# alazarteka/Self-Forcing

Measured on AMD Instinct MI355X. Metric: decoded frames/sec/node, Wan-1.3B 832x480 4-step AR rollout, higher is better.
Workload: dtype bf16

## Files before the change

### self-forcing_amd/csrc/gemm_bf16.hip

```cpp
#include <type_traits>
#include "sf_common.h"
#include "lds_dma.h"
#include "../../include/sf_hip.h"

namespace {

constexpr int BM = 128, BN = 128, BK = 64;
constexpr int GEMM_THREADS = 256;
constexpr int TILE_BYTES = BM * BK * 2;
constexpr int STAGE_BYTES = 2 * TILE_BYTES;
constexpr int GEMM_LDS = 2 * STAGE_BYTES;

struct GemmP {
  const bf16_t* a;
  const bf16_t* w;
  const bf16_t* bias;
  bf16_t* out;
  const bf16_t* resid;
  const bf16_t* gate_mod;
  const bf16_t* gate_e0;
  long gate_group_stride;
  int rows_per_group;
  int M, N, K, lda, ldw, ldo, ldr;
  int tiles_m, tiles_n;
  long a_bs, w_bs, o_bs, r_bs;
  const float* a_scale;
  const float* w_scale;
  int rows_per_seg;
};

typedef int i32x4 __attribute__((ext_vector_type(4)));
typedef int i32x8 __attribute__((ext_vector_type(8)));

__device__ __forceinline__ f32x4 mfma_f8(const bf16x8& w0, const bf16x8& w1, const bf16x8& x0, const bf16x8& x1, const f32x4& acc) {
  const i32x8 wv = __builtin_shufflevector(__builtin_bit_cast(i32x4, w0), __builtin_bit_cast(i32x4, w1), 0, 1, 2, 3, 4, 5, 6, 7);
  const i32x8 xv = __builtin_shufflevector(__builtin_bit_cast(i32x4, x0), __builtin_bit_cast(i32x4, x1), 0, 1, 2, 3, 4, 5, 6, 7);
  return __builtin_amdgcn_mfma_scale_f32_16x16x128_f8f6f4(wv, xv, acc, 0, 0, 0, 127, 0, 127);
}

template <int MT>
__device__ __forceinline__ void fp8_scale_acc(const GemmP& p, f32x4 (&acc)[MT][4], int m_base, int n_base, int lane) {
  f32x4 ws[4];
#pragma unroll
  for (int nt = 0; nt < 4; ++nt) ws[nt] = *reinterpret_cast<const f32x4*>(p.w_scale + min(n_base + nt * 16 + (lane >> 4) * 4, p.N - 4));
#pragma unroll
  for (int mt = 0; mt < MT; ++mt) {
    const float sa = p.a_scale[min(m_base + mt * 16 + (lane & 15), p.M - 1) / p.rows_per_seg];
#pragma unroll
    for (int nt = 0; nt < 4; ++nt)
#pragma unroll
      for (int j = 0; j < 4; ++j) acc[mt][nt][j] = acc[mt][nt][j] * (sa * ws[nt][j]);
  }
}

template <int EPI>
__device__ __forceinline__ bf16x4 epi_apply(const GemmP& p, const f32x4& a4, int m, int n, const bf16_t* e0row) {
  float y[4];
#pragma unroll
  for (int j = 0; j < 4; ++j) y[j] = a4[j];
  if (p.bias) {
    const bf16x4 b = *reinterpret_cast<const bf16x4*>(p.bias + n);
#pragma unroll
    for (int j = 0; j < 4; ++j) y[j] += (float)b[j];
  }
  if (EPI == SF_EPI_BIAS_GELU) {
#pragma unroll
    for (int j = 0; j < 4; ++j) y[j] = gelu_tanh_f(y[j]);
  }
  if (EPI == SF_EPI_BIAS_GATE_RESID) {
    const bf16x4 gm = *reinterpret_cast<const bf16x4*>(p.gate_mod + n);
    const bf16x4 ge = *reinterpret_cast<const bf16x4*>(e0row + n);
#pragma unroll
    for (int j = 0; j < 4; ++j) y[j] *= (float)(bf16_t)((float)gm[j] + (float)ge[j]);
  }
  if (EPI == SF_EPI_BIAS_RESID || EPI == SF_EPI_BIAS_GATE_RESID) {
    const bf16x4 rv = *reinterpret_cast<const bf16x4*>(p.resid + (long)m * p.ldr + n);
#pragma unroll
    for (int j = 0; j < 4; ++j) y[j] += (float)rv[j];
  }
  bf16x4 o;
#pragma unroll
  for (int j = 0; j < 4; ++j) o[j] = (bf16_t)y[j];
  return o;
}

template <int EPI, int MT>
__device__ __forceinline__ void gemm_epilogue(const GemmP& p, f32x4 (&acc)[MT][4], int mrow, int ncol) {
#pragma unroll
  for (int mt = 0; mt < MT; ++mt) {
    const int m = mrow + mt * 16;
    if (m >= p.M) continue;
    const bf16_t* e0row = nullptr;
    if (EPI == SF_EPI_BIAS_GATE_RESID) e0row = p.gate_e0 + (long)(m / p.rows_per_group) * p.gate_group_stride;
#pragma unroll
    for (int nt = 0; nt < 4; ++nt) {
      const int n = ncol + nt * 16;
      if (n >= p.N) continue;
      if (EPI == SF_EPI_F32) {
        *reinterpret_cast<f32x4*>(reinterpret_cast<float*>(p.out) + (long)m * p.ldo + n) = acc[mt][nt];
        continue;
      }
      *reinterpret_cast<bf16x4*>(p.out + (long)m * p.ldo + n) = epi_apply<EPI>(p, acc[mt][nt], m, n, e0row);
    }
  }
}

template <int EPI>
__device__ __forceinline__ bf16x4 epi_math(const f32x4& a4, const bf16x4& b, const bf16x4& gm, const bf16x4& ge, const bf16x4& rv) {
  float y[4];
#pragma unroll
  for (int j = 0; j < 4; ++j) y[j] = a4[j] + (float)b[j];
  if (EPI == SF_EPI_BIAS_GELU) {
#pragma unroll
    for (int j = 0; j < 4; ++j) y[j] = gelu_tanh_f(y[j]);
  }
  if (EPI == SF_EPI_BIAS_GATE_RESID) {
#pragma unroll
    for (int j = 0; j < 4; ++j) y[j] *= (float)(bf16_t)((float)gm[j] + (float)ge[j]);
  }
  if (EPI == SF_EPI_BIAS_RESID || EPI == SF_EPI_BIAS_GATE_RESID) {
#pragma unroll
    for (int j = 0; j < 4; ++j) y[j] += (float)rv[j];
  }
  bf16x4 o;
#pragma unroll
  for (int j = 0; j < 4; ++j) o[j] = (bf16_t)y[j];
  return o;
}

template <int EPI, int MT>
__device__ __forceinline__ void gemm_epilogue_lds(const GemmP& p, f32x4 (&acc)[MT][4], int m_base, int n_base, char* wbuf, int lane) {
  const int r16 = lane & 15, cg = lane >> 4;
  constexpr bool GATE = EPI == SF_EPI_BIAS_GATE_RESID;
  constexpr bool RESID = EPI == SF_EPI_BIAS_RESID || EPI == SF_EPI_BIAS_GATE_RESID;
  const bf16x4 zero4 = {(bf16_t)0.f, (bf16_t)0.f, (bf16_t)0.f, (bf16_t)0.f};
  int ncol[4];
  bf16x4 bias_v[4], gm_v[4];
#pragma unroll
  for (int nt = 0; nt < 4; ++nt) {
    ncol[nt] = min(n_base + nt * 16 + cg * 4, p.N - 4);
    bias_v[nt] = zero4;
    gm_v[nt] = zero4;
  }
  if (p.bias) {
#pragma unroll
    for (int nt = 0; nt < 4; ++nt) bias_v[nt] = *reinterpret_cast<const bf16x4*>(p.bias + ncol[nt]);
  }
  if (GATE) {
#pragma unroll
    for (int nt = 0; nt < 4; ++nt) gm_v[nt] = *reinterpret_cast<const bf16x4*>(p.gate_mod + ncol[nt]);
  }
  constexpr int MB = 4;
#pragma unroll
  for (int m0 = 0; m0 < MT; m0 += MB) {
    bf16x4 rv[MB][4], ge[MB][4];
#pragma unroll
    for (int i = 0; i < MB; ++i) {
      if (m0 + i >= MT) break;
      const int m = min(m_base + (m0 + i) * 16 + r16, p.M - 1);
      const bf16_t* e0row = GATE ? p.gate_e0 + (long)(m / p.rows_per_group) * p.gate_group_stride : nullptr;
#pragma unroll
      for (int nt = 0; nt < 4; ++nt) {
        rv[i][nt] = RESID ? *reinterpret_cast<const bf16x4*>(p.resid + (long)m * p.ldr + ncol[nt]) : zero4;
        ge[i][nt] = GATE ? *reinterpret_cast<const bf16x4*>(e0row + ncol[nt]) : zero4;
      }
    }
#pragma unroll
    for (int i = 0; i < MB; ++i) {
      if (m0 + i >= MT) break;
      const int row = (m0 + i) * 16 + r16;
#pragma unroll
      for (int nt = 0; nt < 4; ++nt) {
        const int col = nt * 16 + cg * 4;
        const bf16x4 o = epi_math<EPI>(acc[m0 + i][nt], bias_v[nt], gm_v[nt], ge[i][nt], rv[i][nt]);
        const int chunk = (col >> 3) ^ (row & 7);
        *reinterpret_cast<bf16x4*>(wbuf + row * 128 + (chunk << 4) + (col & 4) * 2) = o;
      }
    }
  }
  __builtin_amdgcn_s_waitcnt(0xc07f);
  const int rr = lane >> 3, ch = lane & 7;
#pragma unroll
  for (int i = 0; i < 2 * MT; ++i) {
    const int row = i * 8 + rr;
    const int m = m_base + row, n = n_base + ch * 8;
    const bf16x8 v = *reinterpret_cast<const bf16x8*>(wbuf + row * 128 + ((ch ^ (row & 7)) << 4));
    if (m < p.M && n < p.N) *reinterpret_cast<bf16x8*>(p.out + (long)m * p.ldo + n) = v;
  }
}

template <int EPI, bool F8>
__global__ __launch_bounds__(GEMM_THREADS, 2) void gemm_bf16_kernel(GemmP p) {
  extern __shared__ __attribute__((aligned(16))) char smem[];
  const int tid = threadIdx.x;
  const int lane = tid & 63;
  const int wave = __builtin_amdgcn_readfirstlane(tid >> 6);

  if (blockIdx.y) {
    const long bz = blockIdx.y;
    p.a += bz * p.a_bs; p.w += bz * p.w_bs;
    if (EPI == SF_EPI_F32) p.out = reinterpret_cast<bf16_t*>(reinterpret_cast<float*>(p.out) + bz * p.o_bs); else p.out += bz * p.o_bs;
    if (p.resid) p.resid += bz * p.r_bs;
  }
  const int nwg = gridDim.x, bid = blockIdx.x;
  const int wg = sf_xcd_remap(bid, nwg);
  constexpr int GROUP_M = 8;
  const int width = GROUP_M * p.tiles_n;
  const int group = wg / width, first_m = group * GROUP_M;
  const int gsz = min(p.tiles_m - first_m, GROUP_M);
  const int in_group = wg - group * width;
  const int tm = first_m + in_group % gsz, tn = in_group / gsz;
  const int m0 = tm * BM, n0 = tn * BN;

  const bf16_t* a_src[4];
  const bf16_t* w_src[4];
#pragma unroll
  for (int i = 0; i < 4; ++i) {
    const int r = (wave * 4 + i) * 8 + (lane >> 3);
    const int c = (lane & 7) ^ ((r >> 1) & 7);
    const int am = min(m0 + r, p.M - 1);
    const int wn = min(n0 + r, p.N - 1);
    a_src[i] = p.a + (long)am * p.lda + c * 8;
    w_src[i] = p.w + (long)wn * p.ldw + c * 8;
  }
  auto stage = [&](int buf, int kt) {
    char* base = smem + buf * STAGE_BYTES + wave * 4096;
    const int k0 = kt * BK;
#pragma unroll
    for (int i = 0; i < 4; ++i) glds16(a_src[i] + k0, base + i * 1024);
#pragma unroll
    for (int i = 0; i < 4; ++i) glds16(w_src[i] + k0, base + TILE_BYTES + i * 1024);
  };

  const int wr = wave >> 1, wc = wave & 1;
  const int i16 = lane & 15, kq = lane >> 4;
  const int swz = (i16 >> 1) & 7;
  const int x_row_off = (wr * 64 + i16) * 128;
  const int w_row_off = TILE_BYTES + (wc * 64 + i16) * 128;
  const int coff0 = ((0 + kq) ^ swz) << 4;
  const int coff1 = ((4 + kq) ^ swz) << 4;

  f32x4 acc[4][4];
#pragma unroll
  for (int i = 0; i < 4; ++i)
#pragma unroll
    for (int j = 0; j < 4; ++j) acc[i][j] = f32x4{0.f, 0.f, 0.f, 0.f};

  const int nk = p.K / BK;
  stage(0, 0);
  __builtin_amdgcn_s_waitcnt(0);
  __syncthreads();

  for (int kt = 0; kt < nk; ++kt) {
    const int cur = kt & 1;
    const char* buf = smem + cur * STAGE_BYTES;
    const int kn = min(kt + 1, nk - 1) * BK;
    char* sbase = smem + (cur ^ 1) * STAGE_BYTES + wave * 4096;
    bf16x8 xf0[4], wf0[4], xf1[4], wf1[4];
    if constexpr (F8) {
#pragma unroll
      for (int t = 0; t < 4; ++t) {
        xf0[t] = *reinterpret_cast<const bf16x8*>(buf + x_row_off + t * 2048 + coff0);
        wf0[t] = *reinterpret_cast<const bf16x8*>(buf + w_row_off + t * 2048 + coff0);
        xf1[t] = *reinterpret_cast<const bf16x8*>(buf + x_row_off + t * 2048 + coff1);
        wf1[t] = *reinterpret_cast<const bf16x8*>(buf + w_row_off + t * 2048 + coff1);
      }
      __builtin_amdgcn_sched_barrier(0);
#pragma unroll
      for (int i = 0; i < 8; ++i) {
        const int mt = i >> 1, nt0 = (i & 1) * 2;
        acc[mt][nt0] = mfma_f8(wf0[nt0], wf1[nt0], xf0[mt], xf1[mt], acc[mt][nt0]);
        acc[mt][nt0 + 1] = mfma_f8(wf0[nt0 + 1], wf1[nt0 + 1], xf0[mt], xf1[mt], acc[mt][nt0 + 1]);
        if (i < 4) glds16(a_src[i] + kn, sbase + i * 1024);
        else glds16(w_src[i - 4] + kn, sbase + TILE_BYTES + (i - 4) * 1024);
        __builtin_amdgcn_sched_barrier(0);
      }
      __syncthreads();
      continue;
    }
#pragma unroll
    for (int t = 0; t < 4; ++t) {
      xf0[t] = *reinterpret_cast<const bf16x8*>(buf + x_row_off + t * 2048 + coff0);
      wf0[t] = *reinterpret_cast<const bf16x8*>(buf + w_row_off + t * 2048 + coff0);
    }
    __builtin_amdgcn_sched_barrier(0);
#pragma unroll
    for (int i = 0; i < 8; ++i) {
      const int mt = i >> 1, nt0 = (i & 1) * 2;
      acc[mt][nt0] = __builtin_amdgcn_mfma_f32_16x16x32_bf16(wf0[nt0], xf0[mt], acc[mt][nt0], 0, 0, 0);
      acc[mt][nt0 + 1] = __builtin_amdgcn_mfma_f32_16x16x32_bf16(wf0[nt0 + 1], xf0[mt], acc[mt][nt0 + 1], 0, 0, 0);
      if (i < 4) {
        xf1[i] = *reinterpret_cast<const bf16x8*>(buf + x_row_off + i * 2048 + coff1);
        glds16(a_src[i] + kn, sbase + i * 1024);
      } else {
        wf1[i - 4] = *reinterpret_cast<const bf16x8*>(buf + w_row_off + (i - 4) * 2048 + coff1);
        glds16(w_src[i - 4] + kn, sbase + TILE_BYTES + (i - 4) * 1024);
      }
      __builtin_amdgcn_sched_barrier(0);
    }
#pragma unroll
    for (int mt = 0; mt < 4; ++mt)
#pragma unroll
      for (int nt = 0; nt < 4; ++nt)
        acc[mt][nt] = __builtin_amdgcn_mfma_f32_16x16x32_bf16(wf1[nt], xf1[mt], acc[mt][nt], 0, 0, 0);
    __builtin_amdgcn_sched_barrier(0);
    __syncthreads();
  }

  if constexpr (F8) fp8_scale_acc<4>(p, acc, m0 + wr * 64, n0 + wc * 64, lane);
  const int mrow = m0 + wr * 64 + (lane & 15);
  const int ncol = n0 + wc * 64 + (lane >> 4) * 4;
  if (EPI != SF_EPI_F32 && (p.N & 7) == 0 && (p.ldo & 7) == 0)
    gemm_epilogue_lds<EPI, 4>(p, acc, m0 + wr * 64, n0 + wc * 64, smem + wave * 8192, lane);
  else
    gemm_epilogue<EPI, 4>(p, acc, mrow, ncol);
}


constexpr int PP_THREADS = 512;

template <int MT>
struct PPCfg {
  static constexpr int BM = 32 * MT;
  static constexpr int A_BYTES = BM * 128;
  static constexpr int B_BYTES = 256 * 128;
  static constexpr int STAGE = A_BYTES + B_BYTES;
  static constexpr int LDS = 2 * STAGE;
  static constexpr int PA = (2 * MT + 7) / 8;
};

template <int EPI, int MT, bool F8>
__global__ __launch_bounds__(PP_THREADS) void gemm_pp_kernel(GemmP p) {
  using Cfg = PPCfg<MT>;
  constexpr int BMp = Cfg::BM, PA = Cfg::PA;
  constexpr int HQA = (MT + 1) / 2, HQB = MT / 2;
  extern __shared__ __attribute__((aligned(16))) char smem[];
  const int tid = threadIdx.x;
  const int lane = tid & 63;
  const int wave = __builtin_amdgcn_readfirstlane(tid >> 6);
  const int grp = wave >> 2, wc = wave & 3;

  const int nwg = gridDim.x, bid = blockIdx.x;
  const int wg = sf_xcd_remap(bid, nwg);
  constexpr int GROUP_M = MT >= 6 ? 4 : 8;
  const int width = GROUP_M * p.tiles_n;
  const int group = wg / width, first_m = group * GROUP_M;
  const int gsz = min(p.tiles_m - first_m, GROUP_M);
  const int in_group = wg - group * width;
  const int tm = first_m + in_group % gsz, tn = in_group / gsz;
  const int m0 = tm * BMp, n0 = tn * 256;

  const bf16_t* a_src[2][PA];
  const bf16_t* w_src[2][2];
#pragma unroll
  for (int h = 0; h < 2; ++h) {
#pragma unroll
    for (int i = 0; i < PA; ++i) {
      const int r = h * (BMp / 2) + (wave + 8 * i) * 8 + (lane >> 3);
      const int c = (lane & 7) ^ ((r >> 1) & 7);
      a_src[h][i] = p.a + (long)min(m0 + r, p.M - 1) * p.lda + c * 8;
    }
#pragma unroll
    for (int i = 0; i < 2; ++i) {
      const int r = h * 128 + (wave + 8 * i) * 8 + (lane >> 3);
      const int c = (lane & 7) ^ ((r >> 1) & 7);
      w_src[h][i] = p.w + (long)min(n0 + r, p.N - 1) * p.ldw + c * 8;
    }
  }
  auto dma_a = [&](int h, int kt) {
    char* base = smem + (kt & 1) * Cfg::STAGE + h * (Cfg::A_BYTES / 2) + wave * 1024;
#pragma unroll
    for (int i = 0; i < PA; ++i)
      if (wave + 8 * i < 2 * MT) glds16(a_src[h][i] + kt * BK, base + i * 8192);
  };
  auto dma_b = [&](int h, int kt) {
    char* base = smem + (kt & 1) * Cfg::STAGE + Cfg::A_BYTES + h * (Cfg::B_BYTES / 2) + wave * 1024;
#pragma unroll
    for (int i = 0; i < 2; ++i) glds16(w_src[h][i] + kt * BK, base + i * 8192);
  };

  const int i16 = lane & 15, kq = lane >> 4;
  const int swz = (i16 >> 1) & 7;
  const int x_row_off = (grp * (BMp / 2) + i16) * 128;
  const int w_row_off = Cfg::A_BYTES + (wc * 64 + i16) * 128;
  const int coff[2] = {((0 + kq) ^ swz) << 4, ((4 + kq) ^ swz) << 4};

  f32x4 acc[MT][4];
#pragma unroll
  for (int i = 0; i < MT; ++i)
#pragma unroll
    for (int j = 0; j < 4; ++j) acc[i][j] = f32x4{0.f, 0.f, 0.f, 0.f};
  bf16x8 af[HQA][2], bfr[4][2];

#ifdef SF_STAMP
  unsigned long long* stamp = (EPI == SF_EPI_BIAS && p.gate_e0) ? reinterpret_cast<unsigned long long*>(const_cast<bf16_t*>(p.gate_e0)) + ((long)bid * 2 + grp) * 8 : nullptr;
  if (stamp && (tid & 255) == 0) { stamp[0] = __builtin_amdgcn_s_memtime(); stamp[4] = __builtin_amdgcn_s_memrealtime(); }
#endif
  const int nk = p.K / BK;
  dma_a(0, 0); dma_a(1, 0); dma_b(0, 0); dma_b(1, 0);
  if (nk > 1) { dma_b(0, 1); dma_b(1, 1); asm volatile("s_waitcnt vmcnt(4)" ::: "memory"); }
  else asm volatile("s_waitcnt vmcnt(0)" ::: "memory");
  __builtin_amdgcn_s_barrier();
#ifdef SF_STAMP
  if (stamp && (tid & 255) == 0) stamp[1] = __builtin_amdgcn_s_memtime();
#endif
  if (grp == 1) __builtin_amdgcn_s_barrier();

  auto end_load_segment = [&]() {
    __builtin_amdgcn_s_waitcnt(0xc07f);
    __builtin_amdgcn_sched_barrier(0);
    __builtin_amdgcn_s_barrier();
    __builtin_amdgcn_sched_barrier(0);
  };
  auto cluster = [&](auto qc, int c0) {
    constexpr int q = decltype(qc)::value, NQ = q == 0 ? HQA : HQB;
    __builtin_amdgcn_s_setprio(1);
    if constexpr (F8) {
#pragma unroll
      for (int mt = 0; mt < NQ; ++mt)
#pragma unroll
        for (int nt = 0; nt < 2; ++nt)
          acc[q * HQA + mt][c0 + nt] = mfma_f8(bfr[c0 + nt][0], bfr[c0 + nt][1], af[mt][0], af[mt][1], acc[q * HQA + mt][c0 + nt]);
    } else {
#pragma unroll
      for (int ks = 0; ks < 2; ++ks)
#pragma unroll
        for (int mt = 0; mt < NQ; ++mt)
#pragma unroll
          for (int nt = 0; nt < 2; ++nt)
            acc[q * HQA + mt][c0 + nt] = __builtin_amdgcn_mfma_f32_16x16x32_bf16(bfr[c0 + nt][ks], af[mt][ks], acc[q * HQA + mt][c0 + nt], 0, 0, 0);
    }
    __builtin_amdgcn_s_setprio(0);
    __builtin_amdgcn_sched_barrier(0);
    __builtin_amdgcn_s_barrier();
    __builtin_amdgcn_sched_barrier(0);
  };
  auto read_a = [&](const char* buf, auto qc) {
    constexpr int q = decltype(qc)::value, NQ = q == 0 ? HQA : HQB;
#pragma unroll
    for (int mt = 0; mt < NQ; ++mt)
#pragma unroll
      for (int ks = 0; ks < 2; ++ks)
        af[mt][ks] = *reinterpret_cast<const bf16x8*>(buf + x_row_off + (q * HQA + mt) * 2048 + coff[ks]);
  };
  auto read_b = [&](const char* buf, int c0) {
#pragma unroll
    for (int nt = 0; nt < 2; ++nt)
#pragma unroll
      for (int ks = 0; ks < 2; ++ks)
        bfr[c0 + nt][ks] = *reinterpret_cast<const bf16x8*>(buf + w_row_off + (c0 + nt) * 2048 + coff[ks]);
  };

  constexpr std::integral_constant<int, 0> Q0{};
  constexpr std::integral_constant<int, 1> Q1{};
  for (int kt = 0; kt < nk; ++kt) {
    const char* buf = smem + (kt & 1) * Cfg::STAGE;
    const bool more1 = kt + 1 < nk, more2 = kt + 2 < nk;
    read_a(buf, Q0);
    read_b(buf, 0);
    if (more1) dma_a(0, kt + 1);
    end_load_segment();
    cluster(Q0, 0);
    read_b(buf, 2);
    if (more1) dma_a(1, kt + 1);
    end_load_segment();
    cluster(Q0, 2);
    read_a(buf, Q1);
    if (more2) dma_b(0, kt + 2);
    end_load_segment();
    cluster(Q1, 2);
    if (more2) {
      dma_b(1, kt + 2);
      asm volatile("s_waitcnt vmcnt(4)" ::: "memory");
    } else {
      asm volatile("s_waitcnt vmcnt(0)" ::: "memory");
    }
    end_load_segment();
    cluster(Q1, 0);
  }
  if (grp == 0) __builtin_amdgcn_s_barrier();
#ifdef SF_STAMP
  if (stamp && (tid & 255) == 0) stamp[2] = __builtin_amdgcn_s_memtime();
#endif

  const int m_base = m0 + grp * (BMp / 2), n_base = n0 + wc * 64;
  if constexpr (F8) fp8_scale_acc<MT>(p, acc, m_base, n_base, lane);
  if ((p.N & 7) == 0 && (p.ldo & 7) == 0)
    gemm_epilogue_lds<EPI, MT>(p, acc, m_base, n_base, smem + wave * (MT * 2048), lane);
  else
    gemm_epilogue<EPI, MT>(p, acc, m_base + (lane & 15), n_base + (lane >> 4) * 4);
#ifdef SF_STAMP
  asm volatile("s_waitcnt vmcnt(0)" ::: "memory");
  if (stamp && (tid & 255) == 0) { stamp[3] = __builtin_amdgcn_s_memtime(); stamp[5] = __builtin_amdgcn_s_memrealtime(); }
#endif
}

constexpr int PP2_A = 128 * 128, PP2_B = 256 * 128;
constexpr int PP2_LDS = 3 * (PP2_A + PP2_B);

template <int EPI, bool F8>
__global__ __launch_bounds__(PP_THREADS) void gemm_pp2_kernel(GemmP p) {
  extern __shared__ __attribute__((aligned(16))) char smem[];
  const int tid = threadIdx.x;
  const int lane = tid & 63;
  const int wave = __builtin_amdgcn_readfirstlane(tid >> 6);
  const int grp = wave >> 2, wc = wave & 3;

  const int nwg = gridDim.x, bid = blockIdx.x;
  const int wg = sf_xcd_remap(bid, nwg);
  constexpr int GROUP_M = 8;
  const int width = GROUP_M * p.tiles_n;
  const int group = wg / width, first_m = group * GROUP_M;
  const int gsz = min(p.tiles_m - first_m, GROUP_M);
  const int in_group = wg - group * width;
  const int tm = first_m + in_group % gsz, tn = in_group / gsz;
  const int m0 = tm * 128, n0 = tn * 256;

  const bf16_t* a_src[2];
  const bf16_t* w_src[4];
#pragma unroll
  for (int i = 0; i < 2; ++i) {
    const int r = (wave + 8 * i) * 8 + (lane >> 3);
    a_src[i] = p.a + (long)min(m0 + r, p.M - 1) * p.lda + ((lane & 7) ^ ((r >> 1) & 7)) * 8;
  }
#pragma unroll
  for (int i = 0; i < 4; ++i) {
    const int r = (wave + 8 * i) * 8 + (lane >> 3);
    w_src[i] = p.w + (long)min(n0 + r, p.N - 1) * p.ldw + ((lane & 7) ^ ((r >> 1) & 7)) * 8;
  }
  auto dma_a = [&](int slot, int kt) {
    char* base = smem + slot * PP2_A + wave * 1024;
#pragma unroll
    for (int i = 0; i < 2; ++i) glds16(a_src[i] + kt * BK, base + i * 8192);
  };
  auto dma_b = [&](int slot, int kt) {
    char* base = smem + 3 * PP2_A + slot * PP2_B + wave * 1024;
#pragma unroll
    for (int i = 0; i < 4; ++i) glds16(w_src[i] + kt * BK, base + i * 8192);
  };

  const int i16 = lane & 15, kq = lane >> 4;
  const int swz = (i16 >> 1) & 7;
  const int x_row_off = (grp * 64 + i16) * 128;
  const int w_row_off = 3 * PP2_A + (wc * 64 + i16) * 128;
  const int coff[2] = {((0 + kq) ^ swz) << 4, ((4 + kq) ^ swz) << 4};

  f32x4 acc[4][4];
#pragma unroll
  for (int i = 0; i < 4; ++i)
#pragma unroll
    for (int j = 0; j < 4; ++j) acc[i][j] = f32x4{0.f, 0.f, 0.f, 0.f};
  bf16x8 af[4][2], bfr[4][2];

  const int nk = p.K / BK;
  dma_a(0, 0); dma_b(0, 0);
  if (nk > 1) { dma_a(1, 1); dma_b(1, 1); asm volatile("s_waitcnt vmcnt(6)" ::: "memory"); }
  else asm volatile("s_waitcnt vmcnt(0)" ::: "memory");
  __builtin_amdgcn_s_barrier();
  if (grp == 1) __builtin_amdgcn_s_barrier();

  auto end_load_segment = [&]() {
    __builtin_amdgcn_s_waitcnt(0xc07f);
    __builtin_amdgcn_sched_barrier(0);
    __builtin_amdgcn_s_barrier();
    __builtin_amdgcn_sched_barrier(0);
  };
  auto cluster = [&](int c0) {
    __builtin_amdgcn_s_setprio(1);
    if constexpr (F8) {
#pragma unroll
      for (int mt = 0; mt < 4; ++mt)
#pragma unroll
        for (int nt = 0; nt < 2; ++nt)
          acc[mt][c0 + nt] = mfma_f8(bfr[c0 + nt][0], bfr[c0 + nt][1], af[mt][0], af[mt][1], acc[mt][c0 + nt]);
    } else {
#pragma unroll
      for (int ks = 0; ks < 2; ++ks)
#pragma unroll
        for (int mt = 0; mt < 4; ++mt)
#pragma unroll
          for (int nt = 0; nt < 2; ++nt)
            acc[mt][c0 + nt] = __builtin_amdgcn_mfma_f32_16x16x32_bf16(bfr[c0 + nt][ks], af[mt][ks], acc[mt][c0 + nt], 0, 0, 0);
    }
    __builtin_amdgcn_s_setprio(0);
    __builtin_amdgcn_sched_barrier(0);
    __builtin_amdgcn_s_barrier();
    __builtin_amdgcn_sched_barrier(0);
  };

  int slot = 0;
  for (int kt = 0; kt < nk; ++kt) {
    const char* abuf = smem + slot * PP2_A;
    const char* bbuf = smem + slot * PP2_B;
    const int nslot = slot == 0 ? 2 : slot - 1;
    const bool more2 = kt + 2 < nk;
#pragma unroll
    for (int mt = 0; mt < 4; ++mt)
#pragma unroll
      for (int ks = 0; ks < 2; ++ks) af[mt][ks] = *reinterpret_cast<const bf16x8*>(abuf + x_row_off + mt * 2048 + coff[ks]);
#pragma unroll
    for (int nt = 0; nt < 2; ++nt)
#pragma unroll
      for (int ks = 0; ks < 2; ++ks) bfr[nt][ks] = *reinterpret_cast<const bf16x8*>(bbuf + w_row_off + nt * 2048 + coff[ks]);
    if (more2) dma_a(nslot, kt + 2);
    end_load_segment();
    cluster(0);
#pragma unroll
    for (int nt = 2; nt < 4; ++nt)
#pragma unroll
      for (int ks = 0; ks < 2; ++ks) bfr[nt][ks] = *reinterpret_cast<const bf16x8*>(bbuf + w_row_off + nt * 2048 + coff[ks]);
    if (more2) {
      dma_b(nslot, kt + 2);
      asm volatile("s_waitcnt vmcnt(6)" ::: "memory");
    } else {
      asm volatile("s_waitcnt vmcnt(0)" ::: "memory");
    }
    end_load_segment();
    cluster(2);
    slot = slot == 2 ? 0 : slot + 1;
  }
  if (grp == 0) __builtin_amdgcn_s_barrier();

  const int m_base = m0 + grp * 64, n_base = n0 + wc * 64;
  if constexpr (F8) fp8_scale_acc<4>(p, acc, m_base, n_base, lane);
  if ((p.N & 7) == 0 && (p.ldo & 7) == 0)
    gemm_epilogue_lds<EPI, 4>(p, acc, m_base, n_base, smem + wave * 8192, lane);
  else
    gemm_epilogue<EPI, 4>(p, acc, m_base + (lane & 15), n_base + (lane >> 4) * 4);
}

template <int EPI, bool F8>
int launch_pp2(GemmP& p, hipStream_t s) {
  static bool attr = false;
  if (!attr) {
    (void)hipFuncSetAttribute(reinterpret_cast<const void*>(&gemm_pp2_kernel<EPI, F8>), hipFuncAttributeMaxDynamicSharedMemorySize, PP2_LDS);
    attr = true;
  }
  p.tiles_m = (p.M + 127) / 128;
  p.tiles_n = (p.N + 255) / 256;
  hipLaunchKernelGGL((gemm_pp2_kernel<EPI, F8>), dim3(p.tiles_m * p.tiles_n), dim3(PP_THREADS), PP2_LDS, s, p);
  return 0;
}

template <bool F8>
int launch_pp2_epi(GemmP& p, int epilogue, hipStream_t s) {
  switch (epilogue) {
    case SF_EPI_BIAS: return launch_pp2<SF_EPI_BIAS, F8>(p, s);
    case SF_EPI_BIAS_GELU: return launch_pp2<SF_EPI_BIAS_GELU, F8>(p, s);
    case SF_EPI_BIAS_RESID: return launch_pp2<SF_EPI_BIAS_RESID, F8>(p, s);
    case SF_EPI_BIAS_GATE_RESID: return launch_pp2<SF_EPI_BIAS_GATE_RESID, F8>(p, s);
    default: return -1;
  }
}

template <int EPI, int MT, bool F8>
int launch_pp(GemmP& p, hipStream_t s) {
  using Cfg = PPCfg<MT>;
  static bool attr = false;
  if (!attr) {
    (void)hipFuncSetAttribute(reinterpret_cast<const void*>(&gemm_pp_kernel<EPI, MT, F8>), hipFuncAttributeMaxDynamicSharedMemorySize, Cfg::LDS);
    attr = true;
  }
  p.tiles_m = (p.M + Cfg::BM - 1) / Cfg::BM;
  p.tiles_n = (p.N + 255) / 256;
  hipLaunchKernelGGL((gemm_pp_kernel<EPI, MT, F8>), dim3(p.tiles_m * p.tiles_n), dim3(PP_THREADS), Cfg::LDS, s, p);
  return 0;
}

template <int MT, bool F8>
int launch_pp_epi(GemmP& p, int epilogue, hipStream_t s) {
  switch (epilogue) {
    case SF_EPI_BIAS: return launch_pp<SF_EPI_BIAS, MT, F8>(p, s);
    case SF_EPI_BIAS_GELU: return launch_pp<SF_EPI_BIAS_GELU, MT, F8>(p, s);
    case SF_EPI_BIAS_RESID: return launch_pp<SF_EPI_BIAS_RESID, MT, F8>(p, s);
    case SF_EPI_BIAS_GATE_RESID: return launch_pp<SF_EPI_BIAS_GATE_RESID, MT, F8>(p, s);
    default: return -1;
  }
}

int check_args(const sf_gemm_args* a, const char* name, int bk) {
  SF_CHECK(a != nullptr, "%s: null args", name);
  SF_CHECK(a->M > 0 && a->N > 0 && a->K > 0, "%s: empty problem M=%d N=%d K=%d", name, a->M, a->N, a->K);
  SF_CHECK(a->K % bk == 0, "%s: K=%d must be a multiple of %d", name, a->K, bk);
  SF_CHECK(a->N % 4 == 0, "%s: N=%d must be a multiple of 4", name, a->N);
  SF_CHECK(a->lda % (bk / 8) == 0 && a->ldw % (bk / 8) == 0 && a->ldo % 4 == 0, "%s: lda/ldw must be multiples of %d, ldo of 4", name, bk / 8);
  SF_CHECK(a->lda >= a->K && a->ldw >= a->K && a->ldo >= a->N, "%s: leading dimension too small", name);
  SF_CHECK(a->a && a->w && a->out, "%s: null tensor", name);
  SF_CHECK(((uintptr_t)a->a % 16 == 0) && ((uintptr_t)a->w % 16 == 0) && ((uintptr_t)a->out % 8 == 0), "%s: misaligned tensor", name);
  if (a->epilogue == SF_EPI_BIAS_RESID || a->epilogue == SF_EPI_BIAS_GATE_RESID) {
    SF_CHECK(a->resid != nullptr && a->ldr >= a->N && a->ldr % 4 == 0, "%s: residual epilogue needs resid/ldr", name);
  }
  if (a->epilogue == SF_EPI_BIAS_GATE_RESID) {
    SF_CHECK(a->gate_mod && a->gate_e0 && a->rows_per_group > 0, "%s: gate epilogue needs gate_mod/gate_e0/rows_per_group", name);
  }
  SF_CHECK(a->structure >= SF_GEMM_AUTO && a->structure <= SF_GEMM_PP192, "%s: unknown structure %d", name, a->structure);
  return 0;
}

template <bool F8>
int run_gemm(const sf_gemm_args* a, GemmP& p, const char* name, hipStream_t s) {
  int st = a->structure;
  const int nk = p.K / BK;
  const bool pp_ok = a->batch <= 1 && a->epilogue != SF_EPI_F32 && nk >= 2;
  if (st == SF_GEMM_AUTO) {
    st = SF_GEMM_T128;
    if (pp_ok && a->M >= 1024 && a->N >= 1024 && a->K >= 512) {
      static const struct { int st, rows; double rel; } cand[] = {
          {SF_GEMM_PP256, 256, 1.00}, {SF_GEMM_PP224, 224, 1.02}, {SF_GEMM_PP192, 192, 1.05}, {SF_GEMM_PP128, 128, 1.14}};
      const long tn = (a->N + 255) / 256;
      double best = 1e30;
      for (const auto& c : cand) {
        const long tiles = (long)((a->M + c.rows - 1) / c.rows) * tn;
        const double cost = (double)((tiles + 255) / 256) * (c.rows / 256.0 * c.rel + 0.04);
        if (cost < best - 1e-9) { best = cost; st = c.st; }
      }
    }
  }
  const bool is_pp = st == SF_GEMM_PP256 || st == SF_GEMM_PP224 || st == SF_GEMM_PP192 || st == SF_GEMM_PP128;
  if (is_pp && !pp_ok) st = SF_GEMM_T128;
  else if (is_pp) {
    const int rc = st == SF_GEMM_PP256 ? launch_pp_epi<8, F8>(p, a->epilogue, s)
                 : st == SF_GEMM_PP224 ? launch_pp_epi<7, F8>(p, a->epilogue, s)
                 : st == SF_GEMM_PP192 ? launch_pp_epi<6, F8>(p, a->epilogue, s) : launch_pp2_epi<F8>(p, a->epilogue, s);
    SF_CHECK(rc == 0, "%s: unknown epilogue %d", name, a->epilogue);
    SF_HIP_LAUNCH_CHECK(name);
    return 0;
  }
  const int batch = a->batch > 1 ? a->batch : 1;
  p.a_bs = a->a_bstride; p.w_bs = a->w_bstride; p.o_bs = a->o_bstride; p.r_bs = a->r_bstride;
  SF_CHECK(batch == 1 || (a->a_bstride % 8 == 0 && a->w_bstride % 8 == 0 && a->o_bstride % 4 == 0 && a->r_bstride % 4 == 0),
           "%s: batch strides must keep 16-byte (operands) / 8-byte (output) alignment", name);
  const dim3 grid(p.tiles_m * p.tiles_n, batch), block(GEMM_THREADS);
  switch (a->epilogue) {
    case SF_EPI_BIAS: hipLaunchKernelGGL((gemm_bf16_kernel<SF_EPI_BIAS, F8>), grid, block, GEMM_LDS, s, p); break;
    case SF_EPI_BIAS_GELU: hipLaunchKernelGGL((gemm_bf16_kernel<SF_EPI_BIAS_GELU, F8>), grid, block, GEMM_LDS, s, p); break;
    case SF_EPI_BIAS_RESID: hipLaunchKernelGGL((gemm_bf16_kernel<SF_EPI_BIAS_RESID, F8>), grid, block, GEMM_LDS, s, p); break;
    case SF_EPI_BIAS_GATE_RESID: hipLaunchKernelGGL((gemm_bf16_kernel<SF_EPI_BIAS_GATE_RESID, F8>), grid, block, GEMM_LDS, s, p); break;
    case SF_EPI_F32:
      if constexpr (F8) {
        SF_CHECK(false, "%s: the raw fp32 epilogue is bf16-only", name);
      } else {
        SF_CHECK((uintptr_t)a->out % 16 == 0, "%s: fp32 output must be 16-byte aligned", name);
        hipLaunchKernelGGL((gemm_bf16_kernel<SF_EPI_F32, false>), grid, block, GEMM_LDS, s, p);
      }
      break;
    default: SF_CHECK(false, "%s: unknown epilogue %d", name, a->epilogue);
  }
  SF_HIP_LAUNCH_CHECK(name);
  return 0;
}

void fill_params(const sf_gemm_args* a, GemmP& p, int unit) {
  p.a = (const bf16_t*)a->a; p.w = (const bf16_t*)a->w; p.bias = (const bf16_t*)a->bias;
  p.out = (bf16_t*)a->out; p.resid = (const bf16_t*)a->resid;
  p.gate_mod = (const bf16_t*)a->gate_mod; p.gate_e0 = (const bf16_t*)a->gate_e0;
  p.gate_group_stride = a->gate_group_stride; p.rows_per_group = a->rows_per_group;
  p.M = a->M; p.N = a->N; p.K = a->K / unit; p.lda = a->lda / unit; p.ldw = a->ldw / unit; p.ldo = a->ldo; p.ldr = a->ldr;
  p.tiles_n = (a->N + BN - 1) / BN;
  p.tiles_m = (a->M + BM - 1) / BM;
  p.a_scale = nullptr; p.w_scale = nullptr; p.rows_per_seg = 1;
}

}

extern "C" int sf_gemm_bf16(const sf_gemm_args* a, void* stream) {
  if (const int rc = check_args(a, "sf_gemm_bf16", BK)) return rc;
  GemmP p;
  fill_params(a, p, 1);
  return run_gemm<false>(a, p, "sf_gemm_bf16", (hipStream_t)stream);
}

extern "C" int sf_gemm_fp8(const sf_gemm_args* a, const float* a_scale, int rows_per_segment, const float* w_scale, void* stream) {
  if (const int rc = check_args(a, "sf_gemm_fp8", 2 * BK)) return rc;
  SF_CHECK(a->batch <= 1, "sf_gemm_fp8: batched products are bf16-only");
  SF_CHECK(a_scale && w_scale && rows_per_segment > 0, "sf_gemm_fp8: needs a_scale, w_scale and rows_per_segment > 0");
  SF_CHECK((uintptr_t)w_scale % 16 == 0, "sf_gemm_fp8: w_scale must be 16-byte aligned");
  GemmP p;
  fill_params(a, p, 2);
  p.a_scale = a_scale; p.w_scale = w_scale; p.rows_per_seg = rows_per_segment;
  return run_gemm<true>(a, p, "sf_gemm_fp8", (hipStream_t)stream);
}
```

Measured before the change: 97.15.

## Split GEMM LDS epilogue into halves and optionally overlap with final k-step

Adds helpers that split the LDS-staged epilogue into two halves. All residual and gate loads are issued up front, and the first half's global stores go out while the second half is being computed. Behind a compile-time mask that defaults to off, the pp kernel can peel the last k-iteration and interleave the first half's epilogue with its MFMA clusters, using padded LDS scratch. This is meant to hide epilogue memory latency, at the cost of more registers and possibly higher LDS use.

```diff
diff --git a/self-forcing_amd/csrc/gemm_bf16.hip b/self-forcing_amd/csrc/gemm_bf16.hip
--- a/self-forcing_amd/csrc/gemm_bf16.hip
+++ b/self-forcing_amd/csrc/gemm_bf16.hip
@@ -189,6 +189,104 @@
   }
 }
 
+template <int EPI>
+struct EpiCols {
+  int ncol[4];
+  bf16x4 bias_v[4], gm_v[4];
+};
+
+template <int EPI>
+__device__ __forceinline__ void epi_load_cols(const GemmP& p, int n_base, int lane, EpiCols<EPI>& c) {
+  const bf16x4 zero4 = {(bf16_t)0.f, (bf16_t)0.f, (bf16_t)0.f, (bf16_t)0.f};
+#pragma unroll
+  for (int nt = 0; nt < 4; ++nt) {
+    c.ncol[nt] = min(n_base + nt * 16 + (lane >> 4) * 4, p.N - 4);
+    c.bias_v[nt] = zero4;
+    c.gm_v[nt] = zero4;
+  }
+  if (p.bias) {
+#pragma unroll
+    for (int nt = 0; nt < 4; ++nt) c.bias_v[nt] = *reinterpret_cast<const bf16x4*>(p.bias + c.ncol[nt]);
+  }
+  if (EPI == SF_EPI_BIAS_GATE_RESID) {
+#pragma unroll
+    for (int nt = 0; nt < 4; ++nt) c.gm_v[nt] = *reinterpret_cast<const bf16x4*>(p.gate_mod + c.ncol[nt]);
+  }
+}
+
+template <int EPI, int NT>
+__device__ __forceinline__ void epi_load_rows(const GemmP& p, const EpiCols<EPI>& c, int m_base, int t0, int lane,
+                                              bf16x4 (&rv)[NT][4], bf16x4 (&ge)[NT][4]) {
+  constexpr bool GATE = EPI == SF_EPI_BIAS_GATE_RESID;
+  constexpr bool RESID = EPI == SF_EPI_BIAS_RESID || EPI == SF_EPI_BIAS_GATE_RESID;
+  const bf16x4 zero4 = {(bf16_t)0.f, (bf16_t)0.f, (bf16_t)0.f, (bf16_t)0.f};
+#pragma unroll
+  for (int i = 0; i < NT; ++i) {
+    const int m = min(m_base + (t0 + i) * 16 + (lane & 15), p.M - 1);
+    const bf16_t* e0row = GATE ? p.gate_e0 + (long)(m / p.rows_per_group) * p.gate_group_stride : nullptr;
+#pragma unroll
+    for (int nt = 0; nt < 4; ++nt) {
+      rv[i][nt] = RESID ? *reinterpret_cast<const bf16x4*>(p.resid + (long)m * p.ldr + c.ncol[nt]) : zero4;
+      ge[i][nt] = GATE ? *reinterpret_cast<const bf16x4*>(e0row + c.ncol[nt]) : zero4;
+    }
+  }
+}
+
+template <int EPI, int MT, int NT>
+__device__ __forceinline__ void epi_write_rows(const f32x4 (&acc)[MT][4], int t0, const EpiCols<EPI>& c, const bf16x4 (&rv)[NT][4],
+                                               const bf16x4 (&ge)[NT][4], char* wbuf, int lane) {
+  const int r16 = lane & 15, cg = lane >> 4;
+#pragma unroll
+  for (int i = 0; i < NT; ++i) {
+    const int row = i * 16 + r16;
+#pragma unroll
+    for (int nt = 0; nt < 4; ++nt) {
+      const int col = nt * 16 + cg * 4;
+      const bf16x4 o = epi_math<EPI>(acc[t0 + i][nt], c.bias_v[nt], c.gm_v[nt], ge[i][nt], rv[i][nt]);
+      const int chunk = (col >> 3) ^ (row & 7);
+      *reinterpret_cast<bf16x4*>(wbuf + row * 128 + (chunk << 4) + (col & 4) * 2) = o;
+    }
+  }
+}
+
+template <int NT>
+__device__ __forceinline__ void epi_store_rows(const GemmP& p, const char* wbuf, int m_base, int n_base, int t0, int lane) {
+  const int rr = lane >> 3, ch = lane & 7;
+  bf16x8 v[2 * NT];
+#pragma unroll
+  for (int i = 0; i < 2 * NT; ++i) {
+    const int row = i * 8 + rr;
+    v[i] = *reinterpret_cast<const bf16x8*>(wbuf + row * 128 + ((ch ^ (row & 7)) << 4));
+  }
+#pragma unroll
+  for (int i = 0; i < 2 * NT; ++i) {
+    const int m = m_base + t0 * 16 + i * 8 + rr, n = n_base + ch * 8;
+    if (m < p.M && n < p.N) *reinterpret_cast<bf16x8*>(p.out + (long)m * p.ldo + n) = v[i];
+  }
+}
+
+template <int EPI, int MT, int T0, int T1>
+__device__ __forceinline__ void epi_lds_range(const GemmP& p, const f32x4 (&acc)[MT][4], const EpiCols<EPI>& c, int m_base, int n_base,
+                                              char* wbuf, int lane, unsigned long long* stamp = nullptr) {
+  constexpr int H0 = (T1 - T0 + 1) / 2, H1 = T1 - T0 - H0;
+  static_assert(H1 > 0, "two halves");
+  bf16x4 rv0[H0][4], ge0[H0][4], rv1[H1][4], ge1[H1][4];
+  epi_load_rows<EPI, H0>(p, c, m_base, T0, lane, rv0, ge0);
+  epi_load_rows<EPI, H1>(p, c, m_base, T0 + H0, lane, rv1, ge1);
+  epi_write_rows<EPI, MT, H0>(acc, T0, c, rv0, ge0, wbuf, lane);
+  __builtin_amdgcn_s_waitcnt(0xc07f);
+  epi_store_rows<H0>(p, wbuf, m_base, n_base, T0, lane);
+  epi_write_rows<EPI, MT, H1>(acc, T0 + H0, c, rv1, ge1, wbuf + H0 * 2048, lane);
+  __builtin_amdgcn_s_waitcnt(0xc07f);
+#ifdef SF_STAMP
+  if (stamp) stamp[6] = __builtin_amdgcn_s_memtime();
+#endif
+  epi_store_rows<H1>(p, wbuf + H0 * 2048, m_base, n_base, T0 + H0, lane);
+#ifdef SF_STAMP
+  if (stamp) stamp[7] = __builtin_amdgcn_s_memtime();
+#endif
+}
+
 template <int EPI, bool F8>
 __global__ __launch_bounds__(GEMM_THREADS, 2) void gemm_bf16_kernel(GemmP p) {
   extern __shared__ __attribute__((aligned(16))) char smem[];
@@ -319,13 +417,23 @@
 
 constexpr int PP_THREADS = 512;
 
+#ifndef SF_PP_EARLY_MASK
+#define SF_PP_EARLY_MASK 0
+#endif
+template <int EPI, int MT, bool F8>
+constexpr bool pp_early = !F8 && ((SF_PP_EARLY_MASK >> EPI) & 1) != 0 &&
+                          (EPI == SF_EPI_BIAS || EPI == SF_EPI_BIAS_GELU || (EPI == SF_EPI_BIAS_RESID && MT <= 7));
+
 template <int MT>
 struct PPCfg {
   static constexpr int BM = 32 * MT;
   static constexpr int A_BYTES = BM * 128;
   static constexpr int B_BYTES = 256 * 128;
   static constexpr int STAGE = A_BYTES + B_BYTES;
-  static constexpr int LDS = 2 * STAGE;
+  static constexpr int HQA = (MT + 1) / 2;
+  static constexpr int EARLY = 8 * HQA * 2048;
+  static constexpr int PAD = (SF_PP_EARLY_MASK != 0 && EARLY > STAGE) ? EARLY - STAGE : 0;
+  static constexpr int LDS = 2 * STAGE + 2 * PAD;
   static constexpr int PA = (2 * MT + 7) / 8;
 };
 
@@ -334,7 +442,9 @@
   using Cfg = PPCfg<MT>;
   constexpr int BMp = Cfg::BM, PA = Cfg::PA;
   constexpr int HQA = (MT + 1) / 2, HQB = MT / 2;
+  constexpr bool EARLY = pp_early<EPI, MT, F8>;
   extern __shared__ __attribute__((aligned(16))) char smem[];
+  char* const stages = smem + Cfg::PAD;
   const int tid = threadIdx.x;
   const int lane = tid & 63;
   const int wave = __builtin_amdgcn_readfirstlane(tid >> 6);
@@ -368,13 +478,13 @@
     }
   }
   auto dma_a = [&](int h, int kt) {
-    char* base = smem + (kt & 1) * Cfg::STAGE + h * (Cfg::A_BYTES / 2) + wave * 1024;
+    char* base = stages + (kt & 1) * Cfg::STAGE + h * (Cfg::A_BYTES / 2) + wave * 1024;
 #pragma unroll
     for (int i = 0; i < PA; ++i)
       if (wave + 8 * i < 2 * MT) glds16(a_src[h][i] + kt * BK, base + i * 8192);
   };
   auto dma_b = [&](int h, int kt) {
-    char* base = smem + (kt & 1) * Cfg::STAGE + Cfg::A_BYTES + h * (Cfg::B_BYTES / 2) + wave * 1024;
+    char* base = stages + (kt & 1) * Cfg::STAGE + Cfg::A_BYTES + h * (Cfg::B_BYTES / 2) + wave * 1024;
 #pragma unroll
     for (int i = 0; i < 2; ++i) glds16(w_src[h][i] + kt * BK, base + i * 8192);
   };
@@ -393,7 +503,7 @@
   bf16x8 af[HQA][2], bfr[4][2];
 
 #ifdef SF_STAMP
-  unsigned long long* stamp = (EPI == SF_EPI_BIAS && p.gate_e0) ? reinterpret_cast<unsigned long long*>(const_cast<bf16_t*>(p.gate_e0)) + ((long)bid * 2 + grp) * 8 : nullptr;
+  unsigned long long* stamp = (EPI != SF_EPI_BIAS_GATE_RESID && p.gate_e0) ? reinterpret_cast<unsigned long long*>(const_cast<bf16_t*>(p.gate_e0)) + ((long)bid * 2 + grp) * 8 : nullptr;
   if (stamp && (tid & 255) == 0) { stamp[0] = __builtin_amdgcn_s_memtime(); stamp[4] = __builtin_amdgcn_s_memrealtime(); }
 #endif
   const int nk = p.K / BK;
@@ -453,8 +563,12 @@
 
   constexpr std::integral_constant<int, 0> Q0{};
   constexpr std::integral_constant<int, 1> Q1{};
-  for (int kt = 0; kt < nk; ++kt) {
-    const char* buf = smem + (kt & 1) * Cfg::STAGE;
+  const int m_base = m0 + grp * (BMp / 2), n_base = n0 + wc * 64;
+  const bool lds_epi = (p.N & 7) == 0 && (p.ldo & 7) == 0;
+  const bool early = EARLY && lds_epi;
+  const int nk_loop = EARLY ? nk - 1 : nk;
+  for (int kt = 0; kt < nk_loop; ++kt) {
+    const char* buf = stages + (kt & 1) * Cfg::STAGE;
     const bool more1 = kt + 1 < nk, more2 = kt + 2 < nk;
     read_a(buf, Q0);
     read_b(buf, 0);
@@ -478,20 +592,58 @@
     end_load_segment();
     cluster(Q1, 0);
   }
+  EpiCols<EPI> ec;
+  if constexpr (EARLY) {
+    const char* buf = stages + ((nk - 1) & 1) * Cfg::STAGE;
+    char* escr = smem + (((nk - 1) & 1) ? 0 : Cfg::LDS - Cfg::EARLY) + wave * (HQA * 2048);
+    bf16x4 erv[HQA][4], ege[HQA][4];
+    read_a(buf, Q0);
+    read_b(buf, 0);
+    if (early) {
+      epi_load_cols<EPI>(p, n_base, lane, ec);
+      epi_load_rows<EPI, HQA>(p, ec, m_base, 0, lane, erv, ege);
+    }
+    end_load_segment();
+    cluster(Q0, 0);
+    read_b(buf, 2);
+    end_load_segment();
+    cluster(Q0, 2);
+    read_a(buf, Q1);
+    if (early) epi_write_rows<EPI, MT, HQA>(acc, 0, ec, erv, ege, escr, lane);
+    end_load_segment();
+    cluster(Q1, 2);
+    if (early) epi_store_rows<HQA>(p, escr, m_base, n_base, 0, lane);
+    else asm volatile("s_waitcnt vmcnt(0)" ::: "memory");
+    end_load_segment();
+    cluster(Q1, 0);
+  }
   if (grp == 0) __builtin_amdgcn_s_barrier();
 #ifdef SF_STAMP
-  if (stamp && (tid & 255) == 0) stamp[2] = __builtin_amdgcn_s_memtime();
+  const bool stamper = stamp && (tid & 255) == 0;
+  if (stamper) stamp[2] = __builtin_amdgcn_s_memtime();
+  unsigned long long* const estamp = stamper ? stamp : nullptr;
+#else
+  unsigned long long* const estamp = nullptr;
 #endif
 
-  const int m_base = m0 + grp * (BMp / 2), n_base = n0 + wc * 64;
-  if constexpr (F8) fp8_scale_acc<MT>(p, acc, m_base, n_base, lane);
-  if ((p.N & 7) == 0 && (p.ldo & 7) == 0)
-    gemm_epilogue_lds<EPI, MT>(p, acc, m_base, n_base, smem + wave * (MT * 2048), lane);
-  else
-    gemm_epilogue<EPI, MT>(p, acc, m_base + (lane & 15), n_base + (lane >> 4) * 4);
+  if (early) {
+    if constexpr (EARLY) epi_lds_range<EPI, MT, HQA, MT>(p, acc, ec, m_base, n_base, smem + wave * (HQB * 2048), lane, estamp);
+  } else {
+    if constexpr (F8) fp8_scale_acc<MT>(p, acc, m_base, n_base, lane);
+    if (lds_epi) {
+      if constexpr ((EPI == SF_EPI_BIAS_RESID || EPI == SF_EPI_BIAS_GATE_RESID) && MT >= 7) {
+        gemm_epilogue_lds<EPI, MT>(p, acc, m_base, n_base, smem + wave * (MT * 2048), lane);
+      } else {
+        epi_load_cols<EPI>(p, n_base, lane, ec);
+        epi_lds_range<EPI, MT, 0, MT>(p, acc, ec, m_base, n_base, smem + wave * (MT * 2048), lane, estamp);
+      }
+    } else {
+      gemm_epilogue<EPI, MT>(p, acc, m_base + (lane & 15), n_base + (lane >> 4) * 4);
+    }
+  }
 #ifdef SF_STAMP
   asm volatile("s_waitcnt vmcnt(0)" ::: "memory");
-  if (stamp && (tid & 255) == 0) { stamp[3] = __builtin_amdgcn_s_memtime(); stamp[5] = __builtin_amdgcn_s_memrealtime(); }
+  if (stamper) { stamp[3] = __builtin_amdgcn_s_memtime(); stamp[5] = __builtin_amdgcn_s_memrealtime(); }
 #endif
 }
 
@@ -623,10 +775,13 @@
 
   const int m_base = m0 + grp * 64, n_base = n0 + wc * 64;
   if constexpr (F8) fp8_scale_acc<4>(p, acc, m_base, n_base, lane);
-  if ((p.N & 7) == 0 && (p.ldo & 7) == 0)
-    gemm_epilogue_lds<EPI, 4>(p, acc, m_base, n_base, smem + wave * 8192, lane);
-  else
+  if ((p.N & 7) == 0 && (p.ldo & 7) == 0) {
+    EpiCols<EPI> ec;
+    epi_load_cols<EPI>(p, n_base, lane, ec);
+    epi_lds_range<EPI, 4, 0, 4>(p, acc, ec, m_base, n_base, smem + wave * 8192, lane);
+  } else {
     gemm_epilogue<EPI, 4>(p, acc, m_base + (lane & 15), n_base + (lane >> 4) * 4);
+  }
 }
 
 template <int EPI, bool F8>
```

Result: no change. 97.27, median of 4 (+0.1%).
